# akvas/grates

Hardware: NVIDIA B200
Metric: sh_synthesis_grid_points_x_epochs_per_s (higher is better)
Workload: dtype f64

## Files before the change

### grates_b200/csrc/gb_synthesis.cu

```cuda
#include <type_traits>
#include <vector>
#include "gb_common.cuh"
#include "gb_gemm.cuh"

#ifdef GB_TRACE
__device__ unsigned long long gb_trace_buf[2][160][24][2];
#define GB_TRACE_MARK(k, slot)                                                                      \
    do {                                                                                            \
        unsigned long long gt_;                                                                     \
        asm volatile("mov.u64 %0, %%globaltimer;" : "=l"(gt_));                                      \
        if (blockIdx.x < 160 && (slot) < 24) {                                                      \
            gb_trace_buf[k][blockIdx.x][slot][0] = gt_;                                             \
            gb_trace_buf[k][blockIdx.x][slot][1] = (unsigned long long)clock64();                   \
        }                                                                                           \
    } while (0)
#else
#define GB_TRACE_MARK(k, slot) ((void)0)
#endif

namespace {

using gb::legendre_column;

constexpr int S1_TI = 32;
// ... 11 lines not shown
    if (tid < S1_TI) {
        const int i = i0 + tid;
        if (i < nlat) {
            const double* kn_i = kn + (size_t)i * L + m;
            legendre_column(m, L, ct[i], pmm[(size_t)i * L + m], ra, rb, rc,
                            [&](int n, double p) { s_pk[(n - m) * S1_TI + tid] = __dmul_rn(p, kn_i[n - m]); });
        } else {
            for (int nn = 0; nn < Kn; ++nn) s_pk[nn * S1_TI + tid] = 0.0;
        }
    }
    __syncthreads();

    const int cols = 2 * E;
    const int lane = tid & 31;
    const int ig = tid >> 5;
    const long long xo = (long long)cols * ((long long)m * L - (long long)m * (m - 1) / 2);
    const double* Xm = X + xo;
    for (int col0 = 0; col0 < cols; col0 += 32) {
        const int col = col0 + lane;
        if (col >= cols) continue;
        double a0 = 0, a1 = 0, a2 = 0, a3 = 0;
        const double* xp = Xm + col;
        const double* pk = s_pk + ig * 4;
#pragma unroll 4
        for (int nn = 0; nn < Kn; ++nn) {
            const double x = __ldg(xp + (size_t)nn * cols);
            const double2 p01 = *reinterpret_cast<const double2*>(pk + nn * S1_TI);
            const double2 p23 = *reinterpret_cast<const double2*>(pk + nn * S1_TI + 2);
            a0 = fma(p01.x, x, a0);
            a1 = fma(p01.y, x, a1);
            a2 = fma(p23.x, x, a2);
            a3 = fma(p23.y, x, a3);
        }
        const int cs = col >= E, e = col - cs * E;
        const int i = i0 + ig * 4;
        const int k = krow[2 * m + cs];
        const long long row = (long long)e * nlat + i;
        if (i + 0 < nlat) AB[gb_ab_offset(row + 0, k, ab_rows)] = a0;
        if (i + 1 < nlat) AB[gb_ab_offset(row + 1, k, ab_rows)] = a1;
        if (i + 2 < nlat) AB[gb_ab_offset(row + 2, k, ab_rows)] = a2;
        if (i + 3 < nlat) AB[gb_ab_offset(row + 3, k, ab_rows)] = a3;
    }
}


constexpr int T1_TM = GB_T1_TM, T1_KC = GB_T1_KC, T1_STAGES = 4;
constexpr int T1_LDA = T1_TM + 4;
__host__ __device__ constexpr int t1_tn(int nwn) { return 40 * nwn; }
__host__ __device__ constexpr int t1_threads(int nwn) { return 32 * (2 * nwn + 3); }
__host__ __device__ constexpr int t1_ctas_per_sm(int nwn) { return nwn <= 2 ? 2 : 1; }
__host__ __device__ constexpr size_t t1_smem(int nwn) {
    return (size_t)T1_STAGES * T1_KC * (T1_LDA + t1_tn(nwn) + 4) * sizeof(double) + 2 * T1_STAGES * sizeof(uint64_t);
}

struct T1Tables {
    const double* ct_pad;
    const double* kn_t;
    const double* pmm_t;
    const double* rec_a;
    const double* rec_b;
    const double* zeros;
    const int* krow;
    int nlat_pad, lpad;
};

template <bool PAIRS, int NWN, bool FOLD>
__global__ void __launch_bounds__(t1_threads(NWN), t1_ctas_per_sm(NWN))
gb_legendre_stage1(const double* __restrict__ X, double* __restrict__ AB, T1Tables tb, int L, int nlat, int E,
                   int ab_rows, int n_lattiles, int n_coltiles, int n_items, int polar) {
    constexpr int T1_TN = t1_tn(NWN), T1_LDB = T1_TN + 4, T1_CONSUMER_WARPS = 2 * NWN;
    constexpr int T1_STAGE_DOUBLES = T1_KC * (T1_LDA + T1_LDB);
    extern __shared__ __align__(128) unsigned char s_raw[];
    double* s_tiles = reinterpret_cast<double*>(s_raw);
    uint64_t* full = reinterpret_cast<uint64_t*>(s_raw + (size_t)T1_STAGES * T1_STAGE_DOUBLES * sizeof(double));
    uint64_t* empty = full + T1_STAGES;
    const int cols = 2 * E;
    const int warp = threadIdx.x >> 5;
    const int lane = threadIdx.x & 31;

    if (threadIdx.x == 0) {
        for (int s = 0; s < T1_STAGES; ++s) {
            gb::mbar_init(&full[s], FOLD ? 2 : 3);
            gb::mbar_init(&empty[s], T1_CONSUMER_WARPS);
        }
        gb::fence_mbar_init();
    }
    __syncthreads();

    int stage = 0;
    uint32_t phase = 0;
    const int tiles_per_pair = n_lattiles * n_coltiles;
    for (int item = blockIdx.x; item < n_items; item += gridDim.x) {
        const int m_first = item / tiles_per_pair;
        const int rem = item - m_first * tiles_per_pair;
        const int i0 = FOLD ? (polar + rem / n_coltiles) * 32 : (rem / n_coltiles) * (polar ? 32 : T1_TM);
        const int i_south = nlat - 64 - i0;
        const int c0 = (rem % n_coltiles) * T1_TN;
        const int m_second = L - 1 - m_first;
        const int npass = (m_second == m_first) ? 1 : 2;
        const int width = min(T1_TN, cols - c0);

        if (warp == T1_CONSUMER_WARPS) {
            for (int pass = 0; pass < npass; ++pass) {
                const int m = pass ? m_second : m_first;
                const int Kn = L - m;
                const int n_chunks = (Kn + T1_KC - 1) / T1_KC;
                const long long xo = (long long)cols * ((long long)m * L - (long long)m * (m - 1) / 2);
                const double* Xm = X + xo + c0;
                for (int c = 0; c < n_chunks; ++c) {
                    const int rows = min(T1_KC, FOLD ? ((Kn - c * T1_KC + 7) & ~7) : ((Kn - c * T1_KC + 3) & ~3));
                    gb::mbar_wait(&empty[stage], phase ^ 1u);
                    double* sB = s_tiles + (size_t)stage * T1_STAGE_DOUBLES + T1_KC * T1_LDA;
                    if (lane == 0) gb::mbar_arrive_expect_tx(&full[stage], (uint32_t)(rows * width * sizeof(double)));
                    __syncwarp();
                    if (lane < rows) {
                        const int nn = c * T1_KC + lane;
                        const double* src = (nn < Kn) ? Xm + (size_t)nn * cols : tb.zeros;
                        gb::bulk_g2s(sB + lane * T1_LDB, src, (uint32_t)(width * sizeof(double)), &full[stage]);
                    }
                    if (++stage == T1_STAGES) { stage = 0; phase ^= 1u; }
                }
            }
        } else if (warp > T1_CONSUMER_WARPS) {
            if (FOLD && warp != T1_CONSUMER_WARPS + 1) continue;
            const int li = (warp - T1_CONSUMER_WARPS - 1) * 32 + lane;
            const int i = (!FOLD && polar && li >= 32) ? i_south + li : i0 + li;
            const double cti = tb.ct_pad[i];
            for (int pass = 0; pass < npass; ++pass) {
                const int m = pass ? m_second : m_first;
                const int n_chunks = (L - m + T1_KC - 1) / T1_KC;
                const double* kn_i = tb.kn_t + (size_t)m * tb.nlat_pad + i;
                const double* c_ra = tb.rec_a + (size_t)m * tb.lpad;
                const double* c_rb = tb.rec_b + (size_t)m * tb.lpad;
                const double seed = tb.pmm_t[(size_t)m * tb.nlat_pad + i];
                double p1 = 0.0, p2 = 0.0;
                for (int c = 0; c < n_chunks; ++c) {
                    double knv[T1_KC], act[T1_KC], rbv[T1_KC];
#pragma unroll
                    for (int kk = 0; kk < T1_KC; ++kk) {
                        const int nn = c * T1_KC + kk;
                        knv[kk] = __ldg(kn_i + (size_t)nn * tb.nlat_pad);
                        act[kk] = __dmul_rn(__ldg(c_ra + nn), cti);
                        rbv[kk] = __ldg(c_rb + nn);
                    }
                    gb::mbar_wait(&empty[stage], phase ^ 1u);
                    double* sA = s_tiles + (size_t)stage * T1_STAGE_DOUBLES + li;
#pragma unroll
                    for (int kk = 0; kk < T1_KC; ++kk) {
                        double pn;
                        if (c == 0 && kk == 0) pn = seed;
                        else pn = __dsub_rn(__dmul_rn(act[kk], p1), __dmul_rn(rbv[kk], p2));
                        p2 = p1;
                        p1 = pn;
                        sA[kk * T1_LDA] = __dmul_rn(pn, knv[kk]);
                    }
                    __syncwarp();
                    if (lane == 0) gb::mbar_arrive(&full[stage]);
                    if (++stage == T1_STAGES) { stage = 0; phase ^= 1u; }
                }
            }
        } else {
            const int wm = warp / NWN;
            const int wn = warp % NWN;
            const int g = lane >> 2, q = lane & 3;
            const bool has_columns = wn * 40 < width;
            if constexpr (FOLD) {
                const int nh = nlat >> 1;
                for (int pass = 0; pass < npass; ++pass) {
                    const int m = pass ? m_second : m_first;
                    const int Kn = L - m;
                    const int n_chunks = (Kn + T1_KC - 1) / T1_KC;
                    double ev[5][2][2], od[5][2][2];
#pragma unroll
                    for (int mi = 0; mi < 5; ++mi)
#pragma unroll
                        for (int ni = 0; ni < 2; ++ni) ev[mi][ni][0] = ev[mi][ni][1] = od[mi][ni][0] = od[mi][ni][1] = 0.0;
                    for (int c = 0; c < n_chunks; ++c) {
                        const int rows = Kn - c * T1_KC;
                        gb::mbar_wait(&full[stage], phase);
                        const double* sP = s_tiles + (size_t)stage * T1_STAGE_DOUBLES + wm * 16 + g;
                        const double* sX = s_tiles + (size_t)stage * T1_STAGE_DOUBLES + T1_KC * T1_LDA + wn * 40 + g;
#pragma unroll
                        for (int kk = 0; kk < T1_KC; kk += 8) {
                            if (kk >= rows || !has_columns) break;
                            double a[5], b[2];
#pragma unroll
                            for (int mi = 0; mi < 5; ++mi) a[mi] = sX[(kk + 2 * q) * T1_LDB + mi * 8];
#pragma unroll
                            for (int ni = 0; ni < 2; ++ni) b[ni] = sP[(kk + 2 * q) * T1_LDA + ni * 8];
#pragma unroll
                            for (int mi = 0; mi < 5; ++mi)
#pragma unroll
                                for (int ni = 0; ni < 2; ++ni) gb::dmma_884(ev[mi][ni][0], ev[mi][ni][1], a[mi], b[ni]);
#pragma unroll
                            for (int mi = 0; mi < 5; ++mi) a[mi] = sX[(kk + 2 * q + 1) * T1_LDB + mi * 8];
#pragma unroll
                            for (int ni = 0; ni < 2; ++ni) b[ni] = sP[(kk + 2 * q + 1) * T1_LDA + ni * 8];
#pragma unroll
                            for (int mi = 0; mi < 5; ++mi)
#pragma unroll
                                for (int ni = 0; ni < 2; ++ni) gb::dmma_884(od[mi][ni][0], od[mi][ni][1], a[mi], b[ni]);
                        }
                        __syncwarp();
                        if (lane == 0) gb::mbar_arrive(&empty[stage]);
                        if (++stage == T1_STAGES) { stage = 0; phase ^= 1u; }
                    }
                    const int kc_row = tb.krow[2 * m], ks_row = tb.krow[2 * m + 1];
                    const int ib = i0 + wm * 16 + 2 * q;
#pragma unroll
                    for (int mi = 0; mi < 5; ++mi) {
                        const int col = c0 + wn * 40 + mi * 8 + g;
                        if (col >= cols) continue;
                        const int cs = col >= E;
                        const int e = col - cs * E;
                        const int k = cs ? ks_row : kc_row;
#pragma unroll
                        for (int ni = 0; ni < 2; ++ni) {
                            const int i = ib + ni * 8;
                            if (i >= nh) continue;
                            const long long rn = (long long)e * nlat + i;
                            const long long rs = (long long)e * nlat + (nlat - 2 - i);
                            gb::st_v2(AB + gb_ab_offset(rn, k, ab_rows), ev[mi][ni][0] + od[mi][ni][0],
                                      ev[mi][ni][1] + od[mi][ni][1]);
                            gb::st_v2(AB + gb_ab_offset(rs, k, ab_rows), ev[mi][ni][1] - od[mi][ni][1],
                                      ev[mi][ni][0] - od[mi][ni][0]);
                        }
                    }
                }
                continue;
            }
            for (int pass = 0; pass < npass; ++pass) {
                const int m = pass ? m_second : m_first;
                const int Kn = L - m;
                const int n_chunks = (Kn + T1_KC - 1) / T1_KC;
                double acc[5][4][2];
#pragma unroll
                for (int mi = 0; mi < 5; ++mi)
#pragma unroll
                    for (int ni = 0; ni < 4; ++ni) acc[mi][ni][0] = acc[mi][ni][1] = 0.0;
                for (int c = 0; c < n_chunks; ++c) {
                    const int rows = Kn - c * T1_KC;
                    gb::mbar_wait(&full[stage], phase);
                    const double* sP = s_tiles + (size_t)stage * T1_STAGE_DOUBLES + wm * 32 + g;
                    const double* sX = s_tiles + (size_t)stage * T1_STAGE_DOUBLES + T1_KC * T1_LDA + wn * 40 + g;
#pragma unroll
                    for (int kk = 0; kk < T1_KC; kk += 4) {
                        if (kk >= rows || !has_columns) break;
                        double a[5], b[4];
#pragma unroll
                        for (int mi = 0; mi < 5; ++mi) a[mi] = sX[(kk + q) * T1_LDB + mi * 8];
#pragma unroll
                        for (int ni = 0; ni < 4; ++ni) b[ni] = sP[(kk + q) * T1_LDA + ni * 8];
#pragma unroll
                        for (int mi = 0; mi < 5; ++mi)
#pragma unroll
                            for (int ni = 0; ni < 4; ++ni) gb::dmma_884(acc[mi][ni][0], acc[mi][ni][1], a[mi], b[ni]);
                    }
                    __syncwarp();
                    if (lane == 0) gb::mbar_arrive(&empty[stage]);
                    if (++stage == T1_STAGES) { stage = 0; phase ^= 1u; }
                }
                const int kc_row = tb.krow[2 * m], ks_row = tb.krow[2 * m + 1];
                const int ib = ((polar && wm) ? i_south : i0) + wm * 32 + 2 * q;
                const int tile_step = ab_rows * GB_LDA - GB_TM;
#pragma unroll
                for (int mi = 0; mi < 5; ++mi) {
                    const int col = c0 + wn * 40 + mi * 8 + g;
                    if (col >= cols) continue;
                    const int cs = col >= E;
                    const int e = col - cs * E;
                    const long long row = (long long)e * nlat + ib;
                    const int o0 = (int)(row & (GB_TM - 1));
                    double* base = AB + ((size_t)(row >> 7) * ab_rows + (cs ? ks_row : kc_row)) * GB_LDA + o0;
#pragma unroll
                    for (int ni = 0; ni < 4; ++ni) {
                        const int i = ib + ni * 8;
                        if (PAIRS) {
                            if (i < nlat)
                                gb::st_v2(base + ni * 8 + ((o0 + ni * 8 >= GB_TM) ? tile_step : 0), acc[mi][ni][0],
                                          acc[mi][ni][1]);
                        } else {
                            if (i < nlat) base[ni * 8 + ((o0 + ni * 8 >= GB_TM) ? tile_step : 0)] = acc[mi][ni][0];
                            if (i + 1 < nlat)
                                base[ni * 8 + 1 + ((o0 + ni * 8 + 1 >= GB_TM) ? tile_step : 0)] = acc[mi][ni][1];
                        }
                    }
                }
            }
        }
    }
}

constexpr int TB_KC = 16;
__host__ __device__ constexpr int tb_lda(bool fold) { return fold ? 36 : 68; }
__host__ __device__ constexpr int tb_ctas_per_sm(int nwn, bool fold) { return nwn <= 2 ? (fold ? 3 : 2) : nwn == 3 ? 2 : 1; }
__host__ __device__ constexpr size_t tb_stage_bytes(int nwn, bool fold) {
    return (size_t)TB_KC * (tb_lda(fold) + t1_tn(nwn) + 4) * sizeof(double);
}
__host__ __device__ constexpr int tb_stages(int nwn, bool fold) {
    const size_t budget = (232448 - 1024 * tb_ctas_per_sm(nwn, fold)) / tb_ctas_per_sm(nwn, fold) - 128;
    const int s = (int)(budget / tb_stage_bytes(nwn, fold));
    return s > 6 ? 6 : s;
}
__host__ __device__ constexpr int tb_threads(int nwn) { return 32 * (2 * nwn + 1); }
__host__ __device__ constexpr size_t tb_smem(int nwn, bool fold) {
    return (size_t)tb_stages(nwn, fold) * tb_stage_bytes(nwn, fold) + 2 * tb_stages(nwn, fold) * sizeof(uint64_t);
}
__host__ __device__ __forceinline__ int tb_fold_row(int nn) { return (nn & ~7) + ((nn & 1) << 2) + ((nn & 7) >> 1); }
__host__ __device__ __forceinline__ int tb_fold_degree(int row) {
    const int r = row & 7;
    return (row & ~7) + (r < 4 ? 2 * r : 2 * (r - 4) + 1);
}

struct TabArgs {
    const double* tab;
    const int* roff;
    long long tile_stride;
    const int* krow;
};

template <bool PAIRS, int NWN, bool FOLD, int MI = 5>
__global__ void __launch_bounds__(tb_threads(NWN), tb_ctas_per_sm(NWN, FOLD))
gb_stage1_tab(const double* __restrict__ X, double* __restrict__ AB, TabArgs tb, int L, int nlat, int E, int ab_rows,
              int n_lattiles, int n_coltiles, int n_items, int polar) {
    constexpr int KC = TB_KC, STAGES = tb_stages(NWN, FOLD);
    static_assert(STAGES >= 2, "the ring needs at least two stages");
    constexpr int TN = 8 * MI * NWN, LDA = tb_lda(FOLD), LDB = TN + 4, CONSUMER_WARPS = 2 * NWN;
    constexpr int STAGE_DOUBLES = KC * (LDA + LDB);
    extern __shared__ __align__(128) unsigned char s_raw[];
    double* s_tiles = reinterpret_cast<double*>(s_raw);
    uint64_t* full = reinterpret_cast<uint64_t*>(s_raw + (size_t)STAGES * STAGE_DOUBLES * sizeof(double));
    uint64_t* empty = full + STAGES;
    const int cols = 2 * E;
    const int warp = threadIdx.x >> 5;
    const int lane = threadIdx.x & 31;

    if (threadIdx.x == 0) {
        GB_TRACE_MARK(0, 0);
        for (int s = 0; s < STAGES; ++s) {
            gb::mbar_init(&full[s], 1);
            gb::mbar_init(&empty[s], CONSUMER_WARPS);
        }
        gb::fence_mbar_init();
    }
    __syncthreads();
    gb::griddep_launch_dependents();
    const int tiles_per_pair = n_lattiles * n_coltiles;
    int n_pre = 0;
    if (warp == CONSUMER_WARPS && lane == 0) {
        for (int item = blockIdx.x; item < n_items && n_pre < STAGES; item += gridDim.x) {
            const int m_first = item / tiles_per_pair;
            const int lt = (item - m_first * tiles_per_pair) / n_coltiles;
            const int m_second = L - 1 - m_first;
            const int npass = (m_second == m_first) ? 1 : 2;
            const double* tab_t = tb.tab + (size_t)lt * tb.tile_stride;
            for (int pass = 0; pass < npass && n_pre < STAGES; ++pass) {
                const int m = pass ? m_second : m_first;
                const int r0 = tb.roff[m], kn_pad = tb.roff[m + 1] - r0;
                for (int r = 0; r < kn_pad && n_pre < STAGES; r += KC, ++n_pre) {
                    const int rows = min(KC, kn_pad - r);
                    gb::mbar_arrive_expect_tx(&full[n_pre], (uint32_t)(rows * (LDB + LDA) * sizeof(double)));
                    gb::bulk_g2s(s_tiles + (size_t)n_pre * STAGE_DOUBLES, tab_t + ((size_t)r0 + r) * LDA,
                                 (uint32_t)(rows * LDA * sizeof(double)), &full[n_pre]);
                }
            }
        }
        gb::griddep_wait();
        GB_TRACE_MARK(0, 1);
    }

    int stage = 0;
    uint32_t phase = 0;
    int chunk_idx = 0;
    for (int item = blockIdx.x; item < n_items; item += gridDim.x) {
        const int m_first = item / tiles_per_pair;
        const int rem = item - m_first * tiles_per_pair;
        const int lt = rem / n_coltiles;
        const int i0 = FOLD ? (polar + lt) * 32 : lt * (polar ? 32 : T1_TM);
        const int i_south = nlat - 64 - i0;
        const int c0 = (rem % n_coltiles) * TN;
        const int m_second = L - 1 - m_first;
        const int npass = (m_second == m_first) ? 1 : 2;
        const int width = min(TN, cols - c0);

        if (warp == CONSUMER_WARPS) {
            if (lane == 0) {
                const double* tab_t = tb.tab + (size_t)lt * tb.tile_stride;
                const int ct = rem % n_coltiles;
                for (int pass = 0; pass < npass; ++pass) {
                    const int m = pass ? m_second : m_first;
                    const int r0 = tb.roff[m], kn_pad = tb.roff[m + 1] - r0;
                    const double* tab_m = tab_t + (size_t)r0 * LDA;
                    const double* x_m = X + ((size_t)r0 * n_coltiles + (size_t)ct * kn_pad) * LDB;
                    for (int r = 0; r < kn_pad; r += KC) {
                        const int rows = min(KC, kn_pad - r);
                        double* sA = s_tiles + (size_t)stage * STAGE_DOUBLES;
                        if (chunk_idx++ >= n_pre) {
                            gb::mbar_wait(&empty[stage], phase ^ 1u);
                            gb::mbar_arrive_expect_tx(&full[stage], (uint32_t)(rows * (LDB + LDA) * sizeof(double)));
                            gb::bulk_g2s(sA, tab_m + (size_t)r * LDA, (uint32_t)(rows * LDA * sizeof(double)), &full[stage]);
                        }
                        gb::bulk_g2s(sA + KC * LDA, x_m + (size_t)r * LDB, (uint32_t)(rows * LDB * sizeof(double)), &full[stage]);
                        if (++stage == STAGES) { stage = 0; phase ^= 1u; }
                    }
                }
            }
        } else {
            const int wm = warp / NWN;
            const int wn = warp % NWN;
            const int g = lane >> 2, q = lane & 3;
            const bool has_columns = wn * (8 * MI) < width;
            if constexpr (FOLD) {
                const int nh = nlat >> 1;
                for (int pass = 0; pass < npass; ++pass) {
                    const int m = pass ? m_second : m_first;
                    const int Kn = L - m;
                    const int n_chunks = (Kn + KC - 1) / KC;
                    const int kc_row = gb::ld_nc_early(tb.krow + 2 * m), ks_row = gb::ld_nc_early(tb.krow + 2 * m + 1);
                    double ev[MI][2][2], od[MI][2][2];
#pragma unroll
                    for (int mi = 0; mi < MI; ++mi)
#pragma unroll
                        for (int ni = 0; ni < 2; ++ni) ev[mi][ni][0] = ev[mi][ni][1] = od[mi][ni][0] = od[mi][ni][1] = 0.0;
                    for (int c = 0; c < n_chunks; ++c) {
                        const int rows = Kn - c * KC;
                        gb::mbar_wait(&full[stage], phase);
#ifdef GB_TRACE
                        if (warp == 0 && lane == 0 && item == (int)blockIdx.x && pass == 0 && c == 0) GB_TRACE_MARK(0, 3);
#endif
                        const double* sP = s_tiles + (size_t)stage * STAGE_DOUBLES + wm * 16 + g;
                        const double* sX = s_tiles + (size_t)stage * STAGE_DOUBLES + KC * LDA + wn * (8 * MI) + g;
#pragma unroll
                        for (int kk = 0; kk < KC; kk += 8) {
                            if (kk >= rows || !has_columns) break;
                            double a[MI], b[2];
#pragma unroll
                            for (int mi = 0; mi < MI; ++mi) a[mi] = sX[(kk + q) * LDB + mi * 8];
#pragma unroll
                            for (int ni = 0; ni < 2; ++ni) b[ni] = sP[(kk + q) * LDA + ni * 8];
#pragma unroll
                            for (int mi = 0; mi < MI; ++mi)
#pragma unroll
                                for (int ni = 0; ni < 2; ++ni) gb::dmma_884(ev[mi][ni][0], ev[mi][ni][1], a[mi], b[ni]);
#pragma unroll
                            for (int mi = 0; mi < MI; ++mi) a[mi] = sX[(kk + 4 + q) * LDB + mi * 8];
#pragma unroll
                            for (int ni = 0; ni < 2; ++ni) b[ni] = sP[(kk + 4 + q) * LDA + ni * 8];
#pragma unroll
                            for (int mi = 0; mi < MI; ++mi)
#pragma unroll
                                for (int ni = 0; ni < 2; ++ni) gb::dmma_884(od[mi][ni][0], od[mi][ni][1], a[mi], b[ni]);
                        }
                        __syncwarp();
                        if (lane == 0) gb::mbar_arrive(&empty[stage]);
                        if (++stage == STAGES) { stage = 0; phase ^= 1u; }
                    }
#ifdef GB_TRACE
                    if (warp == 0 && lane == 0 && item == (int)blockIdx.x) GB_TRACE_MARK(0, 4 + 2 * pass);
#endif
                    int c0e = c0;
                    asm volatile("" : "+r"(c0e));
                    const int ib = i0 + wm * 16 + 4 * q;
                    const bool quads = (nh & 3) == 0;
#pragma unroll
                    for (int mi = 0; mi < MI; ++mi) {
                        const int col = c0e + wn * (8 * MI) + mi * 8 + g;
                        if (col >= cols) continue;
                        const int cs = col >= E;
                        const int e = col - cs * E;
                        const int k = cs ? ks_row : kc_row;
                        if (quads) {
                            if (ib >= nh) continue;
                            const long long rn = (long long)e * nlat + ib;
                            const long long rs = (long long)e * nlat + (nlat - 4 - ib);
                            gb::st_v4(AB + gb_ab_offset(rn, k, ab_rows), ev[mi][0][0] + od[mi][0][0], ev[mi][0][1] + od[mi][0][1],
                                      ev[mi][1][0] + od[mi][1][0], ev[mi][1][1] + od[mi][1][1]);
                            gb::st_v4(AB + gb_ab_offset(rs, k, ab_rows), ev[mi][1][1] - od[mi][1][1], ev[mi][1][0] - od[mi][1][0],
                                      ev[mi][0][1] - od[mi][0][1], ev[mi][0][0] - od[mi][0][0]);
                            continue;
                        }
#pragma unroll
                        for (int ni = 0; ni < 2; ++ni) {
                            const int i = ib + ni * 2;
                            if (i < nh) {
                                const long long rn = (long long)e * nlat + i;
                                gb::st_v2(AB + gb_ab_offset(rn, k, ab_rows), ev[mi][ni][0] + od[mi][ni][0],
                                          ev[mi][ni][1] + od[mi][ni][1]);
                            }
                            if (i + 2 <= nh) {
                                const long long rs = (long long)e * nlat + (nlat - 2 - i);
                                gb::st_v2(AB + gb_ab_offset(rs, k, ab_rows), ev[mi][ni][1] - od[mi][ni][1],
                                          ev[mi][ni][0] - od[mi][ni][0]);
                            }
                        }
                    }
#ifdef GB_TRACE
                    if (warp == 0 && lane == 0 && item == (int)blockIdx.x) GB_TRACE_MARK(0, 5 + 2 * pass);
#endif
                }
                continue;
            }
            for (int pass = 0; pass < npass; ++pass) {
                const int m = pass ? m_second : m_first;
                const int Kn = L - m;
                const int n_chunks = (Kn + KC - 1) / KC;
                const int kc_row = gb::ld_nc_early(tb.krow + 2 * m), ks_row = gb::ld_nc_early(tb.krow + 2 * m + 1);
                double acc[MI][4][2];
#pragma unroll
                for (int mi = 0; mi < MI; ++mi)
#pragma unroll
                    for (int ni = 0; ni < 4; ++ni) acc[mi][ni][0] = acc[mi][ni][1] = 0.0;
                for (int c = 0; c < n_chunks; ++c) {
                    const int rows = (Kn - c * KC + 7) & ~7;
                    gb::mbar_wait(&full[stage], phase);
                    const double* sP = s_tiles + (size_t)stage * STAGE_DOUBLES + wm * 32 + g;
                    const double* sX = s_tiles + (size_t)stage * STAGE_DOUBLES + KC * LDA + wn * (8 * MI) + g;
#pragma unroll
                    for (int kk = 0; kk < KC; kk += 4) {
                        if (kk >= rows || !has_columns) break;
                        double a[MI], b[4];
#pragma unroll
                        for (int mi = 0; mi < MI; ++mi) a[mi] = sX[(kk + q) * LDB + mi * 8];
#pragma unroll
                        for (int ni = 0; ni < 4; ++ni) b[ni] = sP[(kk + q) * LDA + ni * 8];
#pragma unroll
                        for (int mi = 0; mi < MI; ++mi)
#pragma unroll
                            for (int ni = 0; ni < 4; ++ni) gb::dmma_884(acc[mi][ni][0], acc[mi][ni][1], a[mi], b[ni]);
                    }
                    __syncwarp();
                    if (lane == 0) gb::mbar_arrive(&empty[stage]);
                    if (++stage == STAGES) { stage = 0; phase ^= 1u; }
                }
                int c0e = c0;
                asm volatile("" : "+r"(c0e));
                const int ib = ((polar && wm) ? i_south : i0) + wm * 32 + 2 * q;
                const int tile_step = ab_rows * GB_LDA - GB_TM;
#pragma unroll
                for (int mi = 0; mi < MI; ++mi) {
                    const int col = c0e + wn * (8 * MI) + mi * 8 + g;
                    if (col >= cols) continue;
                    const int cs = col >= E;
                    const int e = col - cs * E;
                    const long long row = (long long)e * nlat + ib;
                    const int o0 = (int)(row & (GB_TM - 1));
                    double* base = AB + ((size_t)(row >> 7) * ab_rows + (cs ? ks_row : kc_row)) * GB_LDA + o0;
#pragma unroll
                    for (int ni = 0; ni < 4; ++ni) {
                        const int i = ib + ni * 8;
                        if (PAIRS) {
                            if (i < nlat)
                                gb::st_v2(base + ni * 8 + ((o0 + ni * 8 >= GB_TM) ? tile_step : 0), acc[mi][ni][0],
                                          acc[mi][ni][1]);
                        } else {
                            if (i < nlat) base[ni * 8 + ((o0 + ni * 8 >= GB_TM) ? tile_step : 0)] = acc[mi][ni][0];
                            if (i + 1 < nlat)
                                base[ni * 8 + 1 + ((o0 + ni * 8 + 1 >= GB_TM) ? tile_step : 0)] = acc[mi][ni][1];
                        }
                    }
                }
            }
        }
    }
    if (threadIdx.x == 0) GB_TRACE_MARK(0, 10);
}


__global__ void __launch_bounds__(128)
gb_ptab_kernel(double* __restrict__ tab, const int* __restrict__ roff, long long rtot, int kind, int tile0, int n_tiles,
               int L, int nlat, const double* __restrict__ ct, const double* __restrict__ kn,
               const double* __restrict__ pmm, const double* __restrict__ ra, const double* __restrict__ rb,
               const double* __restrict__ rc) {
    const int per_tile = kind == 0 ? 32 : 64;
    const int lda = kind == 0 ? 36 : 68;
    const long long idx = (long long)blockIdx.x * blockDim.x + threadIdx.x;
    if (idx >= (long long)n_tiles * L * per_tile) return;
    const int li = (int)(idx % per_tile);
    const int m = (int)((idx / per_tile) % L);
    const int t = (int)(idx / ((long long)per_tile * L));
    int i;
    if (kind == 0) {
        const int cc = li & 15;
        i = (tile0 + t) * 32 + (li & 16) + 4 * ((cc & 7) >> 1) + 2 * (cc >> 3) + (cc & 1);
    } else if (kind == 1) {
        i = li < 32 ? t * 32 + li : nlat - 64 - 32 * t + li;
    } else {
        i = t * 64 + li;
    }
    if (i < 0 || i >= nlat) return;
    double* out = tab + ((size_t)t * rtot + roff[m]) * lda + li;
    const double* kn_i = kn + (size_t)i * L;
    legendre_column(m, L, ct[i], pmm[(size_t)i * L + m], ra, rb, rc, [&](int n, double p) {
        const int nn = n - m;
        out[(size_t)tb_fold_row(nn) * lda] = __dmul_rn(p, kn_i[n]);
    });
}

struct RowMajorStore {
    double* out;
    long long M;
    int nlon;
    __device__ __forceinline__ void operator()(long long row, int col, double v0, double v1) const {
        if (row >= M) return;
        double* o = out + (size_t)row * nlon + col;
        if ((nlon & 1) == 0 && col + 1 < nlon) {
            gb::st_cs_v2(o, v0, v1);
        } else {
            if (col < nlon) gb::st_cs(o, v0);
            if (col + 1 < nlon) gb::st_cs(o + 1, v1);
        }
    }
};

constexpr int Q_WM = 4, Q_WN = 2;
constexpr int Q_TM = 32 * Q_WM;
constexpr int Q_TN = 16 * Q_WN;
static_assert(Q_TM == GB_TM && Q_TN == GB_Q_TN, "tile shape must match the tiled HBM layouts");
constexpr int Q_KC = 28;
constexpr int Q_STAGES = 4;
constexpr int Q_LDA = Q_TM + 4;
constexpr int Q_LDB = Q_TN + 4;
constexpr int Q_CONSUMER_WARPS = Q_WM * Q_WN;
constexpr int Q_STAGE_DOUBLES = Q_KC * (Q_LDA + Q_LDB);
constexpr size_t Q_SMEM = (size_t)Q_STAGES * Q_STAGE_DOUBLES * sizeof(double) + (2 * Q_STAGES + 4) * sizeof(uint64_t) + 16;

struct QGroups { int off[5]; };

struct QWork {
    long long n_tiles, n_full;
    int n_ntiles, split, grid;
    __device__ QWork(int n_mtiles, int n_nt, int g) : n_tiles((long long)n_mtiles * n_nt), n_ntiles(n_nt), grid(g) {
        n_full = n_tiles / grid * grid;
        const long long rest = n_tiles - n_full;
        split = rest > 0 && 2 * rest <= grid;
    }
    __device__ bool get(int b, long long i, long long& mt, int& nt, int& half) const {
        long long t = b + i * grid;
        half = -1;
        if (split && t >= n_full) {
            if (t >= n_full + grid) return false;
            const long long j = t - n_full;
            if (j >= 2 * (n_tiles - n_full)) return false;
            t = n_full + (j >> 1);
            half = (int)(j & 1);
        } else if (t >= n_tiles) {
            return false;
        }
        mt = t / n_ntiles;
        nt = (int)(t % n_ntiles);
        return true;
    }
};

constexpr int QE_THREADS = 512;
__global__ void __launch_bounds__(QE_THREADS, 1)
gb_fourier_stage2_sym(const double* __restrict__ AB, int ab_rows, const double* __restrict__ trig_q_t, int kpad_s,
                      QGroups grp, double* __restrict__ out, long long M, int nlon, int nq, int n_mtiles,
                      int n_ntiles, int wide) {
    extern __shared__ __align__(128) unsigned char s_raw[];
    double* s_tiles = reinterpret_cast<double*>(s_raw);
    uint64_t* full = reinterpret_cast<uint64_t*>(s_raw + (size_t)Q_STAGES * Q_STAGE_DOUBLES * sizeof(double));
    uint64_t* empty = full + Q_STAGES;
    uint64_t* tfull = empty + Q_STAGES;
    uint64_t* tempty = tfull + 2;
    uint32_t* s_tmem = reinterpret_cast<uint32_t*>(tempty + 2);
    const int warp = threadIdx.x >> 5;
    const int lane = threadIdx.x & 31;
    constexpr int PRODUCER_WARP = 12;
    if (threadIdx.x == 0) {
        for (int s = 0; s < Q_STAGES; ++s) {
            gb::mbar_init(&full[s], 1);
            gb::mbar_init(&empty[s], Q_CONSUMER_WARPS);
        }
        for (int b = 0; b < 2; ++b) {
            gb::mbar_init(&tfull[b], Q_CONSUMER_WARPS);
            gb::mbar_init(&tempty[b], 4);
        }
        gb::fence_mbar_init();
    }
    if (warp == 0) gb::tmem_alloc(s_tmem, 512);
    gb::tmem_fence_before_sync();
    __syncthreads();
    gb::tmem_fence_after_sync();
    gb::griddep_wait();
    gb::griddep_launch_dependents();

    const QWork work(n_mtiles, n_ntiles, (int)gridDim.x);
    const int h = nlon >> 1;
    auto emit_row = [&](long long row, int jq, const double (&v)[16]) {
        if (row >= M || jq >= nq) return;
        double* orow = out + (size_t)row * nlon;
        double v1[4], v2[4], v3[4], v4[4];
#pragma unroll
        for (int c = 0; c < 4; ++c) {
            const double ce = v[c], co = v[4 + c], se = v[8 + c], so = v[12 + c];
            const double cp = ce + co, cm = ce - co, sp = se + so, sm = se - so;
            v1[c] = cp + sp;
            v2[c] = cm - sm;
            v3[c] = cp - sp;
            v4[c] = cm + sm;
        }
        if (wide && jq + 4 <= nq) {
            gb::st_cs_v4(orow + h + jq, v1[0], v1[1], v1[2], v1[3]);
            gb::st_cs_v4(orow + nlon - 4 - jq, v2[3], v2[2], v2[1], v2[0]);
            gb::st_cs_v4(orow + h - 4 - jq, v3[3], v3[2], v3[1], v3[0]);
            gb::st_cs_v4(orow + jq, v4[0], v4[1], v4[2], v4[3]);
        } else {
#pragma unroll
            for (int c = 0; c < 4; c += 2) {
                const int j = jq + c;
                if (j >= nq) continue;
                gb::st_cs_v2(orow + h + j, v1[c], v1[c + 1]);
                gb::st_cs_v2(orow + nlon - 2 - j, v2[c + 1], v2[c]);
                gb::st_cs_v2(orow + h - 2 - j, v3[c + 1], v3[c]);
                gb::st_cs_v2(orow + j, v4[c], v4[c + 1]);
            }
        }
    };
    auto warp_row0 = [](int wm, int half) { return half < 0 ? wm * 32 : half * 64 + wm * 16; };

    if (warp >= PRODUCER_WARP) {
        asm volatile("setmaxnreg.dec.sync.aligned.u32 40;\n");
        if (warp == PRODUCER_WARP && lane == 0) {
            int stage = 0;
            uint32_t phase = 0;
            long long mt;
            int nt, half;
            for (long long i = 0; work.get(blockIdx.x, i, mt, nt, half); ++i) {
                for (int k0 = 0; k0 < grp.off[4];) {
                    int gend = grp.off[1];
#pragma unroll
                    for (int s = 1; s < 4; ++s)
                        if (k0 >= grp.off[s]) gend = grp.off[s + 1];
                    const int kc = min(Q_KC, gend - k0);
                    gb::mbar_wait(&empty[stage], phase ^ 1u);
                    double* sA = s_tiles + (size_t)stage * Q_STAGE_DOUBLES;
                    double* sB = sA + Q_KC * Q_LDA;
                    const uint32_t bytes_a = (uint32_t)(kc * Q_LDA * sizeof(double));
                    const uint32_t bytes_b = (uint32_t)(kc * Q_LDB * sizeof(double));
                    gb::mbar_arrive_expect_tx(&full[stage], bytes_a + bytes_b);
                    gb::bulk_g2s(sA, AB + ((size_t)mt * ab_rows + k0) * Q_LDA, bytes_a, &full[stage]);
                    gb::bulk_g2s(sB, trig_q_t + ((size_t)nt * kpad_s + k0) * Q_LDB, bytes_b, &full[stage]);
                    if (++stage == Q_STAGES) { stage = 0; phase ^= 1u; }
                    k0 += kc;
                }
            }
        }
    } else if (warp >= Q_CONSUMER_WARPS) {
        asm volatile("setmaxnreg.dec.sync.aligned.u32 104;\n");
        const int sp = warp & 3;
        int tb = 0;
        uint32_t tphase = 0;
        long long mt;
        int nt, half;
        for (long long i = 0; work.get(blockIdx.x, i, mt, nt, half); ++i) {
            gb::mbar_wait(&tfull[tb], tphase);
            gb::tmem_fence_after_sync();
            const int n_slabs = half < 0 ? 4 : 2;
#pragma unroll 1
            for (int cw = 0; cw < 2; ++cw) {
                const int w = sp + 4 * cw;
                const uint32_t taddr = *s_tmem + ((uint32_t)(32 * sp) << 16) + (uint32_t)(tb * 256 + cw * 128);
                const long long row0 = mt * Q_TM + warp_row0(w / Q_WN, half) + (lane >> 2);
                const int jq = nt * Q_TN + (w % Q_WN) * 16 + 4 * (lane & 3);
#pragma unroll 1
                for (int mi = 0; mi < n_slabs; ++mi) {
                    double v[16];
                    gb::tmem_ld16(taddr + 32u * mi, v);
                    emit_row(row0 + mi * 8, jq, v);
                }
            }
            gb::tmem_fence_before_sync();
            __syncwarp();
            if (lane == 0) gb::mbar_arrive(&tempty[tb]);
            if (++tb == 2) { tb = 0; tphase ^= 1u; }
        }
    } else {
        asm volatile("setmaxnreg.inc.sync.aligned.u32 168;\n");
        const int wm = warp / Q_WN;
        const int wn = warp % Q_WN;
        const int g = lane >> 2, q = lane & 3;
        int stage = 0, tb = 0;
        uint32_t phase = 0, tphase = 0;
        auto run_tile = [&](auto mi_tag, int half) {
            constexpr int MI = decltype(mi_tag)::value;
            const int r0 = warp_row0(wm, half);
            double acc[4][MI][2][2];
#pragma unroll
            for (int s = 0; s < 4; ++s)
#pragma unroll
                for (int mi = 0; mi < MI; ++mi)
#pragma unroll
                    for (int ni = 0; ni < 2; ++ni) acc[s][mi][ni][0] = acc[s][mi][ni][1] = 0.0;
#pragma unroll
            for (int s = 0; s < 4; ++s) {
                for (int k0 = grp.off[s]; k0 < grp.off[s + 1];) {
                    const int kc = min(Q_KC, grp.off[s + 1] - k0);
                    gb::mbar_wait(&full[stage], phase);
                    const double* sA = s_tiles + (size_t)stage * Q_STAGE_DOUBLES + r0 + g;
                    const double* sB = s_tiles + (size_t)stage * Q_STAGE_DOUBLES + Q_KC * Q_LDA + wn * 16 + g;
                    auto k_step = [&](int kk) {
                        double a[MI], b[2];
#pragma unroll
                        for (int mi = 0; mi < MI; ++mi) a[mi] = sA[(kk + q) * Q_LDA + mi * 8];
#pragma unroll
                        for (int ni = 0; ni < 2; ++ni) b[ni] = sB[(kk + q) * Q_LDB + ni * 8];
#pragma unroll
                        for (int mi = 0; mi < MI; ++mi)
#pragma unroll
                            for (int ni = 0; ni < 2; ++ni)
                                gb::dmma_884(acc[s][mi][ni][0], acc[s][mi][ni][1], a[mi], b[ni]);
                    };
                    if (kc == Q_KC) {
#pragma unroll
                        for (int kk = 0; kk < Q_KC; kk += 4) k_step(kk);
                    } else {
#pragma unroll
                        for (int kk = 0; kk < Q_KC; kk += 4) {
                            if (kk >= kc) break;
                            k_step(kk);
                        }
                    }
                    __syncwarp();
                    if (lane == 0) gb::mbar_arrive(&empty[stage]);
                    if (++stage == Q_STAGES) { stage = 0; phase ^= 1u; }
                    k0 += kc;
                }
            }
            gb::mbar_wait(&tempty[tb], tphase ^ 1u);
            gb::tmem_fence_after_sync();
            const uint32_t taddr = *s_tmem + ((uint32_t)(32 * (warp & 3)) << 16) + (uint32_t)(tb * 256 + (warp >> 2) * 128);
#pragma unroll
            for (int mi = 0; mi < MI; ++mi) {
                double v[16];
#pragma unroll
                for (int s = 0; s < 4; ++s)
#pragma unroll
                    for (int c = 0; c < 4; ++c) v[4 * s + c] = acc[s][mi][c >> 1][c & 1];
                gb::tmem_st16(taddr + 32u * mi, v);
            }
            gb::tmem_wait_st();
            gb::tmem_fence_before_sync();
            __syncwarp();
            if (lane == 0) gb::mbar_arrive(&tfull[tb]);
            if (++tb == 2) { tb = 0; tphase ^= 1u; }
        };
        long long mt;
        int nt, half;
        for (long long i = 0; work.get(blockIdx.x, i, mt, nt, half); ++i) {
            if (half < 0) run_tile(std::integral_constant<int, 4>{}, half);
            else run_tile(std::integral_constant<int, 2>{}, half);
        }
    }
    gb::tmem_fence_before_sync();
    __syncthreads();
    if (warp == 0) gb::tmem_dealloc(*s_tmem, 512);
}

constexpr int O_KC = 28, O_STAGES = 4;
constexpr int O_STAGE_DOUBLES = O_KC * (Q_LDA + 2 * Q_LDB);
constexpr size_t O_SMEM = (size_t)O_STAGES * O_STAGE_DOUBLES * sizeof(double) + (2 * O_STAGES + 4 * Q_CONSUMER_WARPS) * sizeof(uint64_t) + 16;

struct OGroups { int off[7]; };

__global__ void __launch_bounds__(QE_THREADS, 1)
gb_fourier_stage2_oct(const double* __restrict__ AB, int ab_rows, const double* __restrict__ trig_o_t, int kpad_o, OGroups grp,
                      double* __restrict__ out, long long M, int nlon, int no, int n_mtiles, int n_ntiles, int wide) {
// ... 709 lines not shown
```

Baseline: 253.3 billion.

## Offload stage-1 epilogue stores to dedicated warps via tensor memory staging

For the NWN==6 configuration, consumer warps now write their accumulator fragments into Blackwell tensor memory (TMEM) instead of storing them straight to global AB. Four extra epilogue warps drain the TMEM double buffers and perform the scattered global stores, synchronised by new full/empty mbarriers. This lets the DMMA warps move on to the next pass while earlier results are still being stored. Register budgets are rebalanced with setmaxnreg, and the fragment store logic is pulled into a shared helper. The cost is a 512-column TMEM allocation, more threads per CTA, and extra synchronisation.

```diff
diff --git a/grates_b200/csrc/gb_synthesis.cu b/grates_b200/csrc/gb_synthesis.cu
--- a/grates_b200/csrc/gb_synthesis.cu
+++ b/grates_b200/csrc/gb_synthesis.cu
@@ -337,9 +337,11 @@
     const int s = (int)(budget / tb_stage_bytes(nwn, fold));
     return s > 6 ? 6 : s;
 }
-__host__ __device__ constexpr int tb_threads(int nwn) { return 32 * (2 * nwn + 1); }
+__host__ __device__ constexpr bool tb_epi(int nwn) { return nwn == 6; }
+__host__ __device__ constexpr int tb_threads(int nwn) { return tb_epi(nwn) ? 32 * (2 * nwn + 8) : 32 * (2 * nwn + 1); }
 __host__ __device__ constexpr size_t tb_smem(int nwn, bool fold) {
-    return (size_t)tb_stages(nwn, fold) * tb_stage_bytes(nwn, fold) + 2 * tb_stages(nwn, fold) * sizeof(uint64_t);
+    return (size_t)tb_stages(nwn, fold) * tb_stage_bytes(nwn, fold) + 2 * tb_stages(nwn, fold) * sizeof(uint64_t) +
+           (tb_epi(nwn) ? 2 * 2 * (2 * nwn) * sizeof(uint64_t) + 16 : 0);
 }
 __host__ __device__ __forceinline__ int tb_fold_row(int nn) { return (nn & ~7) + ((nn & 1) << 2) + ((nn & 7) >> 1); }
 __host__ __device__ __forceinline__ int tb_fold_degree(int row) {
@@ -353,6 +355,53 @@
     long long tile_stride;
     const int* krow;
 };
+
+template <bool PAIRS, bool FOLD>
+__device__ __forceinline__ void tb_store_fragment(double* __restrict__ AB, const double (&v)[8], int col, int ib, int kc_row,
+                                                  int ks_row, int nlat, int E, int ab_rows) {
+    if (col >= 2 * E) return;
+    const int cs = col >= E;
+    const int e = col - cs * E;
+    const int k = cs ? ks_row : kc_row;
+    if constexpr (FOLD) {
+        const int nh = nlat >> 1;
+        if ((nh & 3) == 0) {
+            if (ib >= nh) return;
+            const long long rn = (long long)e * nlat + ib;
+            const long long rs = (long long)e * nlat + (nlat - 4 - ib);
+            gb::st_v4(AB + gb_ab_offset(rn, k, ab_rows), v[0], v[1], v[2], v[3]);
+            gb::st_v4(AB + gb_ab_offset(rs, k, ab_rows), v[7], v[6], v[5], v[4]);
+            return;
+        }
+#pragma unroll
+        for (int ni = 0; ni < 2; ++ni) {
+            const int i = ib + ni * 2;
+            if (i < nh) gb::st_v2(AB + gb_ab_offset((long long)e * nlat + i, k, ab_rows), v[2 * ni], v[2 * ni + 1]);
+            if (i + 2 <= nh)
+                gb::st_v2(AB + gb_ab_offset((long long)e * nlat + (nlat - 2 - i), k, ab_rows), v[4 + 2 * ni + 1], v[4 + 2 * ni]);
+        }
+    } else {
+        const long long row = (long long)e * nlat + ib;
+        const int o0 = (int)(row & (GB_TM - 1));
+        const int tile_step = ab_rows * GB_LDA - GB_TM;
+        double* base = AB + ((size_t)(row >> 7) * ab_rows + k) * GB_LDA + o0;
+#pragma unroll
+        for (int ni = 0; ni < 4; ++ni) {
+            const int i = ib + ni * 8;
+            if (PAIRS) {
+                if (i < nlat) gb::st_v2(base + ni * 8 + ((o0 + ni * 8 >= GB_TM) ? tile_step : 0), v[2 * ni], v[2 * ni + 1]);
+            } else {
+                if (i < nlat) base[ni * 8 + ((o0 + ni * 8 >= GB_TM) ? tile_step : 0)] = v[2 * ni];
+                if (i + 1 < nlat) base[ni * 8 + 1 + ((o0 + ni * 8 + 1 >= GB_TM) ? tile_step : 0)] = v[2 * ni + 1];
+            }
+        }
+    }
+}
+
+template <bool FOLD>
+__device__ __forceinline__ int tb_lane_parallel(int wm, int q, int i0, int i_south, int polar) {
+    return FOLD ? i0 + wm * 16 + 4 * q : ((polar && wm) ? i_south : i0) + wm * 32 + 2 * q;
+}
 
 template <bool PAIRS, int NWN, bool FOLD, int MI = 5>
 __global__ void __launch_bounds__(tb_threads(NWN), tb_ctas_per_sm(NWN, FOLD))
@@ -362,10 +411,16 @@
     static_assert(STAGES >= 2, "the ring needs at least two stages");
     constexpr int TN = 8 * MI * NWN, LDA = tb_lda(FOLD), LDB = TN + 4, CONSUMER_WARPS = 2 * NWN;
     constexpr int STAGE_DOUBLES = KC * (LDA + LDB);
+    constexpr bool EPI = tb_epi(NWN);
+    constexpr int T_PASS = 16 * MI, T_BUF = 3 * T_PASS;
+    static_assert(!EPI || (CONSUMER_WARPS == 12 && 2 * T_BUF <= 512), "three consumer warps per lane quarter, two buffers");
     extern __shared__ __align__(128) unsigned char s_raw[];
     double* s_tiles = reinterpret_cast<double*>(s_raw);
     uint64_t* full = reinterpret_cast<uint64_t*>(s_raw + (size_t)STAGES * STAGE_DOUBLES * sizeof(double));
     uint64_t* empty = full + STAGES;
+    uint64_t* tfull = empty + STAGES;
+    uint64_t* tempty = tfull + 2 * CONSUMER_WARPS;
+    uint32_t* s_tmem = reinterpret_cast<uint32_t*>(tempty + 2 * CONSUMER_WARPS);
     const int cols = 2 * E;
     const int warp = threadIdx.x >> 5;
     const int lane = threadIdx.x & 31;
@@ -376,52 +431,108 @@
             gb::mbar_init(&full[s], 1);
             gb::mbar_init(&empty[s], CONSUMER_WARPS);
         }
+        if constexpr (EPI) {
+            for (int b = 0; b < 2 * CONSUMER_WARPS; ++b) {
+                gb::mbar_init(&tfull[b], 1);
+                gb::mbar_init(&tempty[b], 1);
+            }
+        }
         gb::fence_mbar_init();
     }
+    if constexpr (EPI) {
+        if (warp == 0) gb::tmem_alloc(s_tmem, 512);
+        gb::tmem_fence_before_sync();
+    }
     __syncthreads();
+    if constexpr (EPI) gb::tmem_fence_after_sync();
     gb::griddep_launch_dependents();
     const int tiles_per_pair = n_lattiles * n_coltiles;
-    int n_pre = 0;
-    if (warp == CONSUMER_WARPS && lane == 0) {
-        for (int item = blockIdx.x; item < n_items && n_pre < STAGES; item += gridDim.x) {
-            const int m_first = item / tiles_per_pair;
-            const int lt = (item - m_first * tiles_per_pair) / n_coltiles;
-            const int m_second = L - 1 - m_first;
-            const int npass = (m_second == m_first) ? 1 : 2;
-            const double* tab_t = tb.tab + (size_t)lt * tb.tile_stride;
-            for (int pass = 0; pass < npass && n_pre < STAGES; ++pass) {
-                const int m = pass ? m_second : m_first;
-                const int r0 = tb.roff[m], kn_pad = tb.roff[m + 1] - r0;
-                for (int r = 0; r < kn_pad && n_pre < STAGES; r += KC, ++n_pre) {
-                    const int rows = min(KC, kn_pad - r);
-                    gb::mbar_arrive_expect_tx(&full[n_pre], (uint32_t)(rows * (LDB + LDA) * sizeof(double)));
-                    gb::bulk_g2s(s_tiles + (size_t)n_pre * STAGE_DOUBLES, tab_t + ((size_t)r0 + r) * LDA,
-                                 (uint32_t)(rows * LDA * sizeof(double)), &full[n_pre]);
-                }
-            }
-        }
-        gb::griddep_wait();
-        GB_TRACE_MARK(0, 1);
-    }
-
-    int stage = 0;
-    uint32_t phase = 0;
-    int chunk_idx = 0;
-    for (int item = blockIdx.x; item < n_items; item += gridDim.x) {
-        const int m_first = item / tiles_per_pair;
-        const int rem = item - m_first * tiles_per_pair;
-        const int lt = rem / n_coltiles;
-        const int i0 = FOLD ? (polar + lt) * 32 : lt * (polar ? 32 : T1_TM);
-        const int i_south = nlat - 64 - i0;
-        const int c0 = (rem % n_coltiles) * TN;
-        const int m_second = L - 1 - m_first;
-        const int npass = (m_second == m_first) ? 1 : 2;
-        const int width = min(TN, cols - c0);
-
-        if (warp == CONSUMER_WARPS) {
-            if (lane == 0) {
+    struct Item {
+        int m_first, m_second, npass, lt, i0, i_south, c0;
+    };
+    auto item_at = [&](int item) {
+        Item it;
+        it.m_first = item / tiles_per_pair;
+        const int rem = item - it.m_first * tiles_per_pair;
+        it.lt = rem / n_coltiles;
+        it.i0 = FOLD ? (polar + it.lt) * 32 : it.lt * (polar ? 32 : T1_TM);
+        it.i_south = nlat - 64 - it.i0;
+        it.c0 = (rem % n_coltiles) * TN;
+        it.m_second = L - 1 - it.m_first;
+        it.npass = (it.m_second == it.m_first) ? 1 : 2;
+        return it;
+    };
+
+    if (EPI && warp >= CONSUMER_WARPS + 4) {
+        asm volatile("setmaxnreg.dec.sync.aligned.u32 56;\n");
+        const int sp = warp & 3;
+        const int g = lane >> 2, q = lane & 3;
+        const uint32_t t_quarter = *s_tmem + ((uint32_t)(32 * sp) << 16);
+        int tbuf = 0;
+        uint32_t tphase = 0;
+        for (int item = blockIdx.x; item < n_items; item += gridDim.x) {
+            const Item it = item_at(item);
+            for (int pass = 0; pass < it.npass; ++pass) {
+                const int m = pass ? it.m_second : it.m_first;
+                const int kc_row = __ldg(tb.krow + 2 * m), ks_row = __ldg(tb.krow + 2 * m + 1);
+#pragma unroll 1
+                for (int cw = 0; cw < 3; ++cw) {
+                    const int w = sp + 4 * cw;
+                    const int ib = tb_lane_parallel<FOLD>(w / NWN, q, it.i0, it.i_south, polar);
+                    const int col0 = it.c0 + (w % NWN) * (8 * MI) + g;
+                    const uint32_t taddr = t_quarter + (uint32_t)(tbuf * T_BUF + cw * T_PASS);
+                    gb::mbar_wait(&tfull[tbuf * CONSUMER_WARPS + w], tphase);
+                    gb::tmem_fence_after_sync();
+#pragma unroll
+                    for (int mi = 0; mi < MI; ++mi) {
+                        double v[8];
+                        gb::tmem_ld8(taddr + 16u * mi, v);
+                        if (mi == MI - 1) {
+                            gb::tmem_fence_before_sync();
+                            __syncwarp();
+                            if (lane == 0) gb::mbar_arrive(&tempty[tbuf * CONSUMER_WARPS + w]);
+                        }
+                        tb_store_fragment<PAIRS, FOLD>(AB, v, col0 + mi * 8, ib, kc_row, ks_row, nlat, E, ab_rows);
+                    }
+                }
+                if (++tbuf == 2) { tbuf = 0; tphase ^= 1u; }
+            }
+        }
+    } else if (warp >= CONSUMER_WARPS) {
+        if constexpr (EPI) asm volatile("setmaxnreg.dec.sync.aligned.u32 40;\n");
+        if (warp == CONSUMER_WARPS && lane == 0) {
+            int n_pre = 0;
+            for (int item = blockIdx.x; item < n_items && n_pre < STAGES; item += gridDim.x) {
+                const int m_first = item / tiles_per_pair;
+                const int lt = (item - m_first * tiles_per_pair) / n_coltiles;
+                const int m_second = L - 1 - m_first;
+                const int npass = (m_second == m_first) ? 1 : 2;
                 const double* tab_t = tb.tab + (size_t)lt * tb.tile_stride;
+                for (int pass = 0; pass < npass && n_pre < STAGES; ++pass) {
+                    const int m = pass ? m_second : m_first;
+                    const int r0 = tb.roff[m], kn_pad = tb.roff[m + 1] - r0;
+                    for (int r = 0; r < kn_pad && n_pre < STAGES; r += KC, ++n_pre) {
+                        const int rows = min(KC, kn_pad - r);
+                        gb::mbar_arrive_expect_tx(&full[n_pre], (uint32_t)(rows * (LDB + LDA) * sizeof(double)));
+                        gb::bulk_g2s(s_tiles + (size_t)n_pre * STAGE_DOUBLES, tab_t + ((size_t)r0 + r) * LDA,
+                                     (uint32_t)(rows * LDA * sizeof(double)), &full[n_pre]);
+                    }
+                }
+            }
+            gb::griddep_wait();
+            GB_TRACE_MARK(0, 1);
+
+            int stage = 0;
+            uint32_t phase = 0;
+            int chunk_idx = 0;
+            for (int item = blockIdx.x; item < n_items; item += gridDim.x) {
+                const int m_first = item / tiles_per_pair;
+                const int rem = item - m_first * tiles_per_pair;
+                const int lt = rem / n_coltiles;
                 const int ct = rem % n_coltiles;
+                const int m_second = L - 1 - m_first;
+                const int npass = (m_second == m_first) ? 1 : 2;
+                const double* tab_t = tb.tab + (size_t)lt * tb.tile_stride;
                 for (int pass = 0; pass < npass; ++pass) {
                     const int m = pass ? m_second : m_first;
                     const int r0 = tb.roff[m], kn_pad = tb.roff[m + 1] - r0;
@@ -440,18 +551,51 @@
                     }
                 }
             }
-        } else {
-            const int wm = warp / NWN;
-            const int wn = warp % NWN;
-            const int g = lane >> 2, q = lane & 3;
+        }
+    } else {
+        if constexpr (EPI) asm volatile("setmaxnreg.inc.sync.aligned.u32 128;\n");
+        const int wm = warp / NWN;
+        const int wn = warp % NWN;
+        const int g = lane >> 2, q = lane & 3;
+        int stage = 0;
+        uint32_t phase = 0;
+        int tbuf = 0;
+        uint32_t tphase = 0;
+        uint32_t t_mine = 0;
+        if constexpr (EPI) t_mine = *s_tmem + ((uint32_t)(32 * (warp & 3)) << 16) + (uint32_t)((warp >> 2) * T_PASS);
+        auto finish_pass = [&](int c0, int ib, int kc_row, int ks_row, auto&& v_of) {
+            if constexpr (EPI) {
+                gb::mbar_wait(&tempty[tbuf * CONSUMER_WARPS + warp], tphase ^ 1u);
+                gb::tmem_fence_after_sync();
+            }
+            int c0e = c0;
+            asm volatile("" : "+r"(c0e));
+#pragma unroll
+            for (int mi = 0; mi < MI; ++mi) {
+                double v[8];
+                v_of(mi, v);
+                if constexpr (EPI) gb::tmem_st8(t_mine + (uint32_t)(tbuf * T_BUF + 16 * mi), v);
+                else tb_store_fragment<PAIRS, FOLD>(AB, v, c0e + wn * (8 * MI) + mi * 8 + g, ib, kc_row, ks_row, nlat, E, ab_rows);
+            }
+            if constexpr (EPI) {
+                gb::tmem_wait_st();
+                gb::tmem_fence_before_sync();
+                __syncwarp();
+                if (lane == 0) gb::mbar_arrive(&tfull[tbuf * CONSUMER_WARPS + warp]);
+                if (++tbuf == 2) { tbuf = 0; tphase ^= 1u; }
+            }
+        };
+        for (int item = blockIdx.x; item < n_items; item += gridDim.x) {
+            const Item it = item_at(item);
+            const int width = min(TN, cols - it.c0);
             const bool has_columns = wn * (8 * MI) < width;
-            if constexpr (FOLD) {
-                const int nh = nlat >> 1;
-                for (int pass = 0; pass < npass; ++pass) {
-                    const int m = pass ? m_second : m_first;
-                    const int Kn = L - m;
-                    const int n_chunks = (Kn + KC - 1) / KC;
-                    const int kc_row = gb::ld_nc_early(tb.krow + 2 * m), ks_row = gb::ld_nc_early(tb.krow + 2 * m + 1);
+            for (int pass = 0; pass < it.npass; ++pass) {
+                const int m = pass ? it.m_second : it.m_first;
+                const int Kn = L - m;
+                const int n_chunks = (Kn + KC - 1) / KC;
+                const int kc_row = gb::ld_nc_early(tb.krow + 2 * m), ks_row = gb::ld_nc_early(tb.krow + 2 * m + 1);
+                const int ib = tb_lane_parallel<FOLD>(wm, q, it.i0, it.i_south, polar);
+                if constexpr (FOLD) {
                     double ev[MI][2][2], od[MI][2][2];
 #pragma unroll
                     for (int mi = 0; mi < MI; ++mi)
@@ -493,111 +637,63 @@
 #ifdef GB_TRACE
                     if (warp == 0 && lane == 0 && item == (int)blockIdx.x) GB_TRACE_MARK(0, 4 + 2 * pass);
 #endif
-                    int c0e = c0;
-                    asm volatile("" : "+r"(c0e));
-                    const int ib = i0 + wm * 16 + 4 * q;
-                    const bool quads = (nh & 3) == 0;
-#pragma unroll
-                    for (int mi = 0; mi < MI; ++mi) {
-                        const int col = c0e + wn * (8 * MI) + mi * 8 + g;
-                        if (col >= cols) continue;
-                        const int cs = col >= E;
-                        const int e = col - cs * E;
-                        const int k = cs ? ks_row : kc_row;
-                        if (quads) {
-                            if (ib >= nh) continue;
-                            const long long rn = (long long)e * nlat + ib;
-                            const long long rs = (long long)e * nlat + (nlat - 4 - ib);
-                            gb::st_v4(AB + gb_ab_offset(rn, k, ab_rows), ev[mi][0][0] + od[mi][0][0], ev[mi][0][1] + od[mi][0][1],
-                                      ev[mi][1][0] + od[mi][1][0], ev[mi][1][1] + od[mi][1][1]);
-                            gb::st_v4(AB + gb_ab_offset(rs, k, ab_rows), ev[mi][1][1] - od[mi][1][1], ev[mi][1][0] - od[mi][1][0],
-                                      ev[mi][0][1] - od[mi][0][1], ev[mi][0][0] - od[mi][0][0]);
-                            continue;
+                    finish_pass(it.c0, ib, kc_row, ks_row, [&](int mi, double (&v)[8]) {
+#pragma unroll
+                        for (int ni = 0; ni < 2; ++ni)
+#pragma unroll
+                            for (int r = 0; r < 2; ++r) {
+                                v[2 * ni + r] = ev[mi][ni][r] + od[mi][ni][r];
+                                v[4 + 2 * ni + r] = ev[mi][ni][r] - od[mi][ni][r];
+                            }
+                    });
+                } else {
+                    double acc[MI][4][2];
+#pragma unroll
+                    for (int mi = 0; mi < MI; ++mi)
+#pragma unroll
+                        for (int ni = 0; ni < 4; ++ni) acc[mi][ni][0] = acc[mi][ni][1] = 0.0;
+                    for (int c = 0; c < n_chunks; ++c) {
+                        const int rows = (Kn - c * KC + 7) & ~7;
+                        gb::mbar_wait(&full[stage], phase);
+                        const double* sP = s_tiles + (size_t)stage * STAGE_DOUBLES + wm * 32 + g;
+                        const double* sX = s_tiles + (size_t)stage * STAGE_DOUBLES + KC * LDA + wn * (8 * MI) + g;
+#pragma unroll
+                        for (int kk = 0; kk < KC; kk += 4) {
+                            if (kk >= rows || !has_columns) break;
+                            double a[MI], b[4];
+#pragma unroll
+                            for (int mi = 0; mi < MI; ++mi) a[mi] = sX[(kk + q) * LDB + mi * 8];
+#pragma unroll
+                            for (int ni = 0; ni < 4; ++ni) b[ni] = sP[(kk + q) * LDA + ni * 8];
+#pragma unroll
+                            for (int mi = 0; mi < MI; ++mi)
+#pragma unroll
+                                for (int ni = 0; ni < 4; ++ni) gb::dmma_884(acc[mi][ni][0], acc[mi][ni][1], a[mi], b[ni]);
                         }
-#pragma unroll
-                        for (int ni = 0; ni < 2; ++ni) {
-                            const int i = ib + ni * 2;
-                            if (i < nh) {
-                                const long long rn = (long long)e * nlat + i;
-                                gb::st_v2(AB + gb_ab_offset(rn, k, ab_rows), ev[mi][ni][0] + od[mi][ni][0],
-                                          ev[mi][ni][1] + od[mi][ni][1]);
-                            }
-                            if (i + 2 <= nh) {
-                                const long long rs = (long long)e * nlat + (nlat - 2 - i);
-                                gb::st_v2(AB + gb_ab_offset(rs, k, ab_rows), ev[mi][ni][1] - od[mi][ni][1],
-                                          ev[mi][ni][0] - od[mi][ni][0]);
-                            }
+                        __syncwarp();
+                        if (lane == 0) gb::mbar_arrive(&empty[stage]);
+                        if (++stage == STAGES) { stage = 0; phase ^= 1u; }
+                    }
+                    finish_pass(it.c0, ib, kc_row, ks_row, [&](int mi, double (&v)[8]) {
+#pragma unroll
+                        for (int ni = 0; ni < 4; ++ni) {
+                            v[2 * ni] = acc[mi][ni][0];
+                            v[2 * ni + 1] = acc[mi][ni][1];
                         }
-                    }
+                    });
+                }
 #ifdef GB_TRACE
-                    if (warp == 0 && lane == 0 && item == (int)blockIdx.x) GB_TRACE_MARK(0, 5 + 2 * pass);
+                if (warp == 0 && lane == 0 && item == (int)blockIdx.x) GB_TRACE_MARK(0, 5 + 2 * pass);
 #endif
-                }
-                continue;
-            }
-            for (int pass = 0; pass < npass; ++pass) {
-                const int m = pass ? m_second : m_first;
-                const int Kn = L - m;
-                const int n_chunks = (Kn + KC - 1) / KC;
-                const int kc_row = gb::ld_nc_early(tb.krow + 2 * m), ks_row = gb::ld_nc_early(tb.krow + 2 * m + 1);
-                double acc[MI][4][2];
-#pragma unroll
-                for (int mi = 0; mi < MI; ++mi)
-#pragma unroll
-                    for (int ni = 0; ni < 4; ++ni) acc[mi][ni][0] = acc[mi][ni][1] = 0.0;
-                for (int c = 0; c < n_chunks; ++c) {
-                    const int rows = (Kn - c * KC + 7) & ~7;
-                    gb::mbar_wait(&full[stage], phase);
-                    const double* sP = s_tiles + (size_t)stage * STAGE_DOUBLES + wm * 32 + g;
-                    const double* sX = s_tiles + (size_t)stage * STAGE_DOUBLES + KC * LDA + wn * (8 * MI) + g;
-#pragma unroll
-                    for (int kk = 0; kk < KC; kk += 4) {
-                        if (kk >= rows || !has_columns) break;
-                        double a[MI], b[4];
-#pragma unroll
-                        for (int mi = 0; mi < MI; ++mi) a[mi] = sX[(kk + q) * LDB + mi * 8];
-#pragma unroll
-                        for (int ni = 0; ni < 4; ++ni) b[ni] = sP[(kk + q) * LDA + ni * 8];
-#pragma unroll
-                        for (int mi = 0; mi < MI; ++mi)
-#pragma unroll
-                            for (int ni = 0; ni < 4; ++ni) gb::dmma_884(acc[mi][ni][0], acc[mi][ni][1], a[mi], b[ni]);
-                    }
-                    __syncwarp();
-                    if (lane == 0) gb::mbar_arrive(&empty[stage]);
-                    if (++stage == STAGES) { stage = 0; phase ^= 1u; }
-                }
-                int c0e = c0;
-                asm volatile("" : "+r"(c0e));
-                const int ib = ((polar && wm) ? i_south : i0) + wm * 32 + 2 * q;
-                const int tile_step = ab_rows * GB_LDA - GB_TM;
-#pragma unroll
-                for (int mi = 0; mi < MI; ++mi) {
-                    const int col = c0e + wn * (8 * MI) + mi * 8 + g;
-                    if (col >= cols) continue;
-                    const int cs = col >= E;
-                    const int e = col - cs * E;
-                    const long long row = (long long)e * nlat + ib;
-                    const int o0 = (int)(row & (GB_TM - 1));
-                    double* base = AB + ((size_t)(row >> 7) * ab_rows + (cs ? ks_row : kc_row)) * GB_LDA + o0;
-#pragma unroll
-                    for (int ni = 0; ni < 4; ++ni) {
-                        const int i = ib + ni * 8;
-                        if (PAIRS) {
-                            if (i < nlat)
-                                gb::st_v2(base + ni * 8 + ((o0 + ni * 8 >= GB_TM) ? tile_step : 0), acc[mi][ni][0],
-                                          acc[mi][ni][1]);
-                        } else {
-                            if (i < nlat) base[ni * 8 + ((o0 + ni * 8 >= GB_TM) ? tile_step : 0)] = acc[mi][ni][0];
-                            if (i + 1 < nlat)
-                                base[ni * 8 + 1 + ((o0 + ni * 8 + 1 >= GB_TM) ? tile_step : 0)] = acc[mi][ni][1];
-                        }
-                    }
-                }
             }
         }
     }
     if (threadIdx.x == 0) GB_TRACE_MARK(0, 10);
+    if constexpr (EPI) {
+        gb::tmem_fence_before_sync();
+        __syncthreads();
+        if (warp == 0) gb::tmem_dealloc(*s_tmem, 512);
+    }
 }
 
 
```

Result: faster. 258.2 billion, median of 6 (+2.0%).
